# VITA-Group/MM3DGS-SLAM

Measured on AMD Instinct MI355X. Metric: SLAM frames/sec (track+map), TUM fr1/desk-shaped 640x480, higher is better.
Workload: dtype f32

## Files before the change

mm3dgs_slam_amd/csrc/composite.hip:

```cpp
#include <type_traits>
#include "mm3dgs_common.h"
#include "sort_tile.h"
#include "fused_api.h"
#include "loss_pixel.h"
#include "loss_tile.h"

#define STG_ROW 17
#define STG_N (4 * STG_ROW)

#include "composite_common.h"

template <int C>
__device__ __forceinline__ void composite_fwd_body(int tile, const CamDev& cam, const GeomView& g, const ImageView& iv, const BinView& b,
                                                   uint32_t N_cap, float* __restrict__ out, float4 (*stg)[4][3][STG_N],
                                                   const uint32_t* counts_lds, const TrackLoss* tl = nullptr,
                                                   double (*red)[12] = nullptr, const SortShared* span = nullptr) {
  const int tid = threadIdx.x, lane = tid & 63, wv = tid >> 6;
  const int row = lane >> 4, q = lane & 15;
  const int slane = row * STG_ROW + q;
  const int px = (tile % cam.gx) * TILE + (wv & 1) * 8 + (row & 1) * 4 + (q & 3);
  const int py = (tile / cam.gx) * TILE + (wv >> 1) * 8 + (row >> 1) * 4 + (q >> 2);
  const bool inside = px < cam.W && py < cam.H;
  const float pxf = (float)px, pyf = (float)py;
  uint32_t start, len;
// ... 93 lines not shown
#pragma unroll
      for (int k = 0; k < 12; k++) ls[k] = 0.0;
      if (inside) {
        const float rgb[3] = {fin[0], fin[1], fin[2]};
        const float g3[3] = {tl->gt[pix], tl->gt[HW + pix], tl->gt[2 * HW + pix]};
        loss_px_sums(tl->cfg, rgb, fin[4], fin[3], g3, tl->cfg.w_pearson != 0.f ? tl->ref[pix] : 0.f, ls);
      }
      block_sums<12>(ls, red, pearson_double_cols(tl->cfg));
      if (threadIdx.x == 0) {
        double* rowp = tl->partial + (size_t)tile * 12;
#pragma unroll
        for (int k = 0; k < 12; k++) rowp[k] = ls[k];
      }
    }
  }
}

template <int C>
__global__ void __launch_bounds__(256)
composite_fwd_kernel(CamDev cam, GeomView g, ImageView iv, BinView b, uint32_t N_cap, float* __restrict__ out) {
  __shared__ float4 stg[2][4][3][STG_N];
  const int T = cam.gx * cam.gy;
  const int tile = xcd_tile(blockIdx.x, T, cam.tilemap);
  if (tile >= T) return;
  composite_fwd_body<C>(tile, cam, g, iv, b, N_cap, out, stg, nullptr);
}

template <int C>
__global__ void __launch_bounds__(256)
sort_composite_fwd_kernel(CamDev cam, GeomView g, ImageView iv, BinView b, uint32_t N_cap, float* __restrict__ out, int clean, int has_tl,
                          TrackLoss tl, int direct_blocks, uint32_t direct_cap, int slot_bits) {
  __shared__ __align__(16) unsigned char smem[sizeof(float4) * 2 * 4 * 3 * STG_N];
  __shared__ SortShared sh;
  __shared__ double red[4][12];
  static_assert(sizeof(smem) >= 2048 * sizeof(unsigned long long), "LDS union too small for the key array");
  static_assert(sizeof(smem) >= 3 * RANK_SORT_MAX * sizeof(unsigned long long) + sizeof(SortEmit), "LDS union too small for the sort's words and the emission's counters");
  const int T = cam.gx * cam.gy;
  const int tile = slam_tile(cam, iv, blockIdx.x, T);
  if (tile >= T) return;
  sort_tile_body<2048, true>(tile, cam.gx, 0, g, iv, b, N_cap, clean, (unsigned long long*)smem, sh, PROBE_WORD(cam), direct_blocks, direct_cap, slot_bits);
  if (PROBE(cam, 1)) return;
  __syncthreads();
  composite_fwd_body<C>(tile, cam, g, iv, b, N_cap, out, (float4 (*)[4][3][STG_N])smem, sh.run, has_tl ? &tl : nullptr, red, &sh);

}

template <int CTRL>
__device__ __forceinline__ float dpp_all(float v) {
  return __int_as_float(__builtin_amdgcn_update_dpp(0, __float_as_int(v), CTRL, 0xf, 0xf, true));
}
#define QP_XOR1 0xB1
#define QP_XOR2 0x4E
#define ROW_ROR4 0x124
#define ROW_ROR8 0x128

template <int NV>
struct WaveReduce {
  static constexpr int M1 = (NV + 1) / 2;
  static constexpr int M2 = (M1 + 1) / 2;
  static_assert(NV >= 1 && NV <= 16, "NV out of range");
  __device__ static __forceinline__ int slot(int lane) {
    int b0 = lane & 1, b1 = (lane >> 1) & 1, q = (lane >> 2) & 3;
    int i1 = q + M2 * b1;
    int idx = i1 + M1 * b0;
    bool ok = (q < M2) && (i1 < M1) && (idx < NV);
    return ok ? idx : -1;
  }
  __device__ static __forceinline__ float run(const float (&v)[NV], int lane) {
#pragma clang fp contract(off)
    const bool b0 = lane & 1, b1 = lane & 2;
    float l1[M1];
#pragma unroll
    for (int i = 0; i < M1; i++) {
      float sa = v[i] + dpp_all<QP_XOR1>(v[i]);
      if (i + M1 < NV) {
        float sb = v[i + M1] + dpp_all<QP_XOR1>(v[i + M1]);
        l1[i] = b0 ? sb : sa;
      } else {
        l1[i] = sa;
      }
    }
    float l2[M2];
#pragma unroll
    for (int i = 0; i < M2; i++) {
      float sa = l1[i] + dpp_all<QP_XOR2>(l1[i]);
      if (i + M2 < M1) {
        float sb = l1[i + M2] + dpp_all<QP_XOR2>(l1[i + M2]);
        l2[i] = b1 ? sb : sa;
      } else {
        l2[i] = sa;
      }
    }
#pragma unroll
    for (int i = 0; i < M2; i++) {
      l2[i] += dpp_all<ROW_ROR4>(l2[i]);
      l2[i] += dpp_all<ROW_ROR8>(l2[i]);
    }
    const int q = (lane >> 2) & 3;
    float r = l2[0];
#pragma unroll
    for (int i = 1; i < M2; i++) r = (q == i) ? l2[i] : r;
    return r;
  }
};

#define BWD_STG_BYTES (sizeof(float4) * 2 * 4 * 3 * STG_N + sizeof(uint32_t) * 2 * 4 * 64)

constexpr bool bwd_is_two_phase(int MODE, int C) { return MODE != 0 || C == 3; }
#define TP_STRIDE 65
template <int MODE>
struct Bwd2Lds {
  static constexpr int OFF_A = 0;
  static constexpr int OFF_B = OFF_A + STG_N * 16;
  static constexpr int OFF_CZ = OFF_B + STG_N * 16;
  static constexpr int OFF_TP = OFF_CZ + STG_N * 8;
  static constexpr int OFF_T5 = OFF_TP + 4 * TP_STRIDE * 8;
  static constexpr int OFF_T = OFF_TP + 8 * TP_STRIDE * 8;
  static constexpr int SLICE = OFF_T + (MODE == 1 ? 64 * 16 : 64 * 4);
};
template <int MODE>
using BwdLds = Bwd2Lds<(MODE == 0 ? 1 : MODE)>;
template <int C, int MODE>
constexpr size_t BWD_WAVE_SLICE = bwd_is_two_phase(MODE, C) ? (size_t)BwdLds<MODE>::SLICE : sizeof(float4) * 3 * STG_N;
template <int C, int MODE>
constexpr size_t BWD_LDS_BYTES = bwd_is_two_phase(MODE, C) ? 4 * (size_t)BwdLds<MODE>::SLICE : (size_t)BWD_STG_BYTES;
template <int C, int MODE, bool POSE = false>
__device__ __forceinline__ void composite_bwd_body(int tile, const CamDev& cam, const GeomView& g, const ImageView& iv, const BinView& b,
                                                   uint32_t N_cap, const float* __restrict__ dL_dout, float* __restrict__ dsub, int has_tl,
                                                   const TrackLoss& tl, int dl_planes, unsigned char* smem_raw, const SortShared* span = nullptr) {
  static_assert(!POSE || MODE == 2, "the pose chain lives in the tracking mode's loop");
  const int tid = threadIdx.x, lane = tid & 63, wv = tid >> 6;
  const int row = lane >> 4, q = lane & 15;
  const int slane = row * STG_ROW + q;
  const int px = (tile % cam.gx) * TILE + (wv & 1) * 8 + (row & 1) * 4 + (q & 3);
  const int py = (tile / cam.gx) * TILE + (wv >> 1) * 8 + (row >> 1) * 4 + (q >> 2);
  const bool inside = px < cam.W && py < cam.H;
  const float pxf = (float)px, pyf = (float)py;
  uint32_t start, len;
  if (span) { start = span->start; len = span->len; }
  else tile_span(iv, tile, N_cap, start, len);
  const int L = 4 * wv + row;
  const uint32_t count = len ? min(span ? span->run[L] : iv.subcount[NLIST * tile + L], len) : 0u;
  const uint2* __restrict__ list = b.sublist + (size_t)NLIST * start + (size_t)L * len;

  constexpr int NV = MODE == 0 ? 6 + C : (MODE == 1 ? 10 : 7);
  static_assert(MODE == 0 || C == 6, "SLAM modes composite the 6-channel bundle");
  constexpr int RECF = MODE == 0 ? GENERIC_RECF(C) : (MODE == 1 ? REC_MAP_F : REC_TRACK_F);
  float4 (*stg)[4][3][STG_N] = (float4 (*)[4][3][STG_N])smem_raw;
  constexpr uint32_t CH = 16;

  const size_t pix = (size_t)py * cam.W + px, HW = (size_t)cam.H * cam.W;
  const float T_final = inside ? iv.final_T[pix] : 0.f;
  const uint32_t last_contributor = inside ? iv.n_contrib[pix] : 0u;
  uint32_t todo = last_contributor;
  todo = max(todo, (uint32_t)__builtin_amdgcn_update_dpp(0, (int)todo, QP_XOR1, 0xf, 0xf, true));
  todo = max(todo, (uint32_t)__builtin_amdgcn_update_dpp(0, (int)todo, QP_XOR2, 0xf, 0xf, true));
  todo = max(todo, (uint32_t)__builtin_amdgcn_update_dpp(0, (int)todo, ROW_ROR4, 0xf, 0xf, true));
  todo = max(todo, (uint32_t)__builtin_amdgcn_update_dpp(0, (int)todo, ROW_ROR8, 0xf, 0xf, true));
  todo = min(todo, count);
  const uint32_t maxtodo = max(max((uint32_t)__builtin_amdgcn_readlane((int)todo, 0), (uint32_t)__builtin_amdgcn_readlane((int)todo, 16)),
                               max((uint32_t)__builtin_amdgcn_readlane((int)todo, 32), (uint32_t)__builtin_amdgcn_readlane((int)todo, 48)));
  float dL[C];
  float bg_dot = 0.f;
  bool dl_done = false;
  if constexpr (MODE == 2) {
    if (has_tl) {
#pragma unroll
      for (int ch = 0; ch < C; ch++) dL[ch] = 0.f;
      if (inside) {
        const float sil = tl.out[4 * HW + pix];
        const bool smask = sil > tl.cfg.sil_thr;
        const float l1s = tl.defer_scale ? tl.cfg.w_l1 / 3.f : loss_l1_scale(tl.cfg, tl.sums);
#pragma unroll
        for (int ch = 0; ch < 3; ch++) dL[ch] = loss_px_l1_grad(tl.cfg, tl.out[ch * HW + pix], tl.gt[ch * HW + pix], smask, l1s);
        if (tl.cfg.w_pearson != 0.f) dL[3] = loss_px_pearson_grad(tl.cfg, sil, tl.out[3 * HW + pix], tl.ref[pix], tl.sums);
      }
      if (!tl.defer_scale && tile == 0 && threadIdx.x == 0 && tl.loss4) loss_scalars(tl.cfg, tl.sums, HW, tl.loss4);
      dl_done = true;
    }
  }
  if constexpr (MODE == 1) {
    if (has_tl) {
      LossGradSmem& lsm = *(LossGradSmem*)smem_raw;
      float* exch = (float*)(smem_raw + sizeof(LossGradSmem));
      float g4[4];
      bool in_raster;
      if (PROBE(cam, 10)) { g4[0] = g4[1] = g4[2] = g4[3] = 1e-3f; in_raster = true; }
      else loss_grad_tile(tl.cfg, tl.out, tl.gt, tl.ref, tl.dmaps, tl.sums, tile, cam.gx, lsm, g4, in_raster);
#pragma unroll
      for (int ch = 0; ch < 4; ch++) exch[ch * 256 + tid] = g4[ch];
      __syncthreads();
      const int lx = (wv & 1) * 8 + (row & 1) * 4 + (q & 3), ly = (wv >> 1) * 8 + (row >> 1) * 4 + (q >> 2);
#pragma unroll
      for (int ch = 0; ch < C; ch++) dL[ch] = ch < 4 ? exch[ch * 256 + ly * 16 + lx] : 0.f;
      __syncthreads();
      dl_done = true;
    }
  }
#pragma unroll
  for (int ch = 0; ch < C; ch++) {
    if (!dl_done) dL[ch] = (inside && ch < dl_planes) ? dL_dout[ch * HW + pix] : 0.f;
    if (ch < 3 || cam.bg_extras) bg_dot += cam.bg[ch % 3] * dL[ch];
  }
  const float Tf_bg = T_final * bg_dot;
  float Tr = T_final;
  float behind_dot = 0.f;

  const size_t rbase = (size_t)NLIST * start + (size_t)L * len;
  if constexpr (!POSE)
  for (uint32_t e = todo + q; e < count; e += 16) {
    zero_record<NV>(dsub + (rbase + e) * RECF);
  }
  float pacc[6] = {0.f, 0.f, 0.f, 0.f, 0.f, 0.f};
  if constexpr (bwd_is_two_phase(MODE, C)) {
  if (maxtodo != 0) {
    using LY = BwdLds<MODE>;
    unsigned char* const wbase = smem_raw + (size_t)wv * LY::SLICE;
    float4* const sA = (float4*)(wbase + LY::OFF_A);
    float4* const sB = (float4*)(wbase + LY::OFF_B);
    float2* const sCZ = (float2*)(wbase + LY::OFF_CZ);
    float2* const tp = (float2*)(wbase + LY::OFF_TP);
    float* const t5 = (float*)(wbase + LY::OFF_T5);
    bool z45_wave = true;
    if constexpr (MODE == 0) ((float4*)(wbase + LY::OFF_T))[lane] = make_float4(dL[0], dL[1], dL[2], 0.f);
    else {
      if constexpr (MODE == 1) ((float4*)(wbase + LY::OFF_T))[lane] = make_float4(dL[0], dL[1], dL[C > 3 ? 2 : 0], dL[C > 3 ? 3 : 0]);
      else ((float*)(wbase + LY::OFF_T))[lane] = dL[C > 3 ? 3 : 0];
      z45_wave = __ballot(dL[C > 4 ? 4 : 0] != 0.f || dL[C > 5 ? 5 : 0] != 0.f || Tf_bg != 0.f) == 0ull;
      if (!z45_wave) t5[lane] = dL[C > 5 ? 5 : 0];
    }
    const uint32_t first_step = todo - min(todo, last_contributor);
    const uint32_t mean_steps_b = wave_mean_steps(cam, iv);
    const float X0 = pxf - (float)(q & 3), Y0 = pyf - (float)(q >> 2);
    uint32_t n_visit = 0;
    uint32_t my_idx;
    {
      const uint2 e0 = (uint32_t)q < todo ? list[todo - 1u - q] : make_uint2(0u, 0u);
      const SplatRec r0 = load_rec<C>(g.splat, e0.x, (uint32_t)q < todo);
      sA[slane] = r0.A; sB[slane] = r0.B; sCZ[slane] = make_float2(r0.C.x, r0.C.y);
      my_idx = POSE ? e0.x : e0.y;
    }
    uint2 ent_nxt = CH + q < todo ? list[todo - 1u - (CH + q)] : make_uint2(0u, 0u);
    auto run2 = [&](auto z45_tag) {
      constexpr bool Z45 = decltype(z45_tag)::value;
      constexpr int SUB = Z45 ? 8 : 4;
      constexpr int NL = 16 / SUB;
      const int e = q & (SUB - 1), part = q / SUB;
      const int r17 = row * STG_ROW;
      for (uint32_t base = 0; base < maxtodo; base += CH) {
        const SplatRec rec_n = load_rec<C>(g.splat, ent_nxt.x, base + CH + q < todo);
        const uint2 ent_nn = base + 2 * CH + q < todo ? list[todo - 1u - (base + 2 * CH + q)] : make_uint2(0u, 0u);
        __builtin_amdgcn_wave_barrier();
        const int cnt = __builtin_amdgcn_readfirstlane((int)min(CH, maxtodo - base));
        for (int sub = 0; sub < cnt; sub += SUB) {
          const int cs = min(SUB, cnt - sub);
          float2* tpw = tp + lane;
          auto splat_px = [&](const float4& A, const float4& B, const float2& CZ, const int j) {
            const uint32_t step = base + (uint32_t)j;
            const bool row_on = step < todo;
            const float dx = A.x - pxf, dy = A.y - pyf;
            const float power = splat_power(dx, dy, A.z, A.w, B.x);
            const float G = SPLAT_EXP(power);
            const float alpha = fminf(0.99f, B.y * G);
            const bool valid = row_on && (step >= first_step) && !(power > 0.f) && !(alpha < ALPHA_MIN);
            n_visit++;
            const float a_eff = valid ? alpha : 0.f;
            const float G_eff = valid ? G : 0.f;
            float r;
            if constexpr (MODE == 0) {
              const float d = 1.f - a_eff, r0 = __builtin_amdgcn_rcpf(d);
              r = fmaf(fmaf(-d, r0, 1.f), r0, r0);
            } else r = __builtin_amdgcn_rcpf(1.f - a_eff);
            Tr *= r;
            const float w = a_eff * Tr;
            float qd = fmaf(B.z, dL[0], 0.f);
            qd = fmaf(B.w, dL[1], qd);
            qd = fmaf(CZ.x, dL[2], qd);
            if constexpr (MODE != 0) qd = fmaf(CZ.y, dL[C > 3 ? 3 : 0], qd);
            if constexpr (!Z45 && MODE != 0) { qd = fmaf(1.f, dL[C > 4 ? 4 : 0], qd); qd = fmaf(CZ.y * CZ.y, dL[C > 5 ? 5 : 0], qd); }
            const float diff = qd - behind_dot;
            behind_dot = fmaf(a_eff, diff, behind_dot);
            const float dLa = (Z45 && MODE != 0) ? diff * Tr : diff * Tr - Tf_bg * r;
            const float u = MODE == 0 ? dLa * G_eff : B.y * dLa * G_eff;
            *tpw = make_float2(u, w);
            tpw += TP_STRIDE;
          };
          {
            float4 A0 = sA[r17 + sub], B0 = sB[r17 + sub];
            float2 Z0 = sCZ[r17 + sub];
            for (int j = sub; j < sub + cs; j += 2) {
              const int j1 = j + 1 < sub + cs ? j + 1 : j;
              const float4 A1 = sA[r17 + j1], B1 = sB[r17 + j1];
              const float2 Z1 = sCZ[r17 + j1];
              splat_px(A0, B0, Z0, j);
              if (j + 1 < sub + cs) {
                const int j2 = j + 2 < sub + cs ? j + 2 : j1;
                A0 = sA[r17 + j2]; B0 = sB[r17 + j2]; Z0 = sCZ[r17 + j2];
                splat_px(A1, B1, Z1, j1);
              }
            }
          }
          __builtin_amdgcn_wave_barrier();
          {
#pragma clang fp contract(off)
            const int ent = sub + e;
            const bool on2 = base + (uint32_t)ent < todo;
            const float2 cxy = *(const float2*)&sA[r17 + ent];
            const uint32_t idx = (uint32_t)__builtin_amdgcn_ds_bpermute((row * 16 + ent) << 2, (int)my_idx);
            float4 k0, k1, k2, k3, k4;
            if constexpr (POSE) {
              const float4* pr = (const float4*)(g.poserec + (size_t)(on2 ? idx : 0u) * POSEREC_F);
              k0 = pr[0]; k1 = pr[1]; k2 = pr[2]; k3 = pr[3]; k4 = pr[4];
            }
            float dxv[4], dxx[4];
#pragma unroll
            for (int x = 0; x < 4; x++) { dxv[x] = cxy.x - (X0 + (float)x); dxx[x] = dxv[x] * dxv[x]; }
            float M0 = 0.f, Mx = 0.f, Mxx = 0.f, My = 0.f, Mxy = 0.f, Myy = 0.f, c0 = 0.f, c1 = 0.f, c2 = 0.f, cz = 0.f, cz5 = 0.f;
            const float2* tpr = tp + e * TP_STRIDE + row * 16 + part * SUB;
            const int pcol = row * 16 + part * SUB;
#pragma unroll
            for (int yy = 0; yy < SUB / 4; yy++) {
              float s0 = 0.f, s1 = 0.f, s2 = 0.f;
#pragma unroll
              for (int x = 0; x < 4; x++) {
                const float2 uw = tpr[yy * 4 + x];
                s0 = s0 + uw.x;
                s1 = __builtin_fmaf(uw.x, dxv[x], s1);
                s2 = __builtin_fmaf(uw.x, dxx[x], s2);
                if constexpr (MODE != 2) {
                  const float4 d4 = ((const float4*)(wbase + LY::OFF_T))[pcol + yy * 4 + x];
                  c0 = __builtin_fmaf(uw.y, d4.x, c0);
                  c1 = __builtin_fmaf(uw.y, d4.y, c1);
                  c2 = __builtin_fmaf(uw.y, d4.z, c2);
                  if constexpr (MODE == 1) cz = __builtin_fmaf(uw.y, d4.w, cz);
                } else {
                  cz = __builtin_fmaf(uw.y, ((const float*)(wbase + LY::OFF_T))[pcol + yy * 4 + x], cz);
                }
                if constexpr (!Z45) cz5 = __builtin_fmaf(uw.y, t5[pcol + yy * 4 + x], cz5);
              }
              const float dyv = cxy.y - (Y0 + (float)(part * (SUB / 4) + yy));
              M0 = M0 + s0; Mx = Mx + s1; Mxx = Mxx + s2;
              My = __builtin_fmaf(s0, dyv, My);
              Mxy = __builtin_fmaf(s1, dyv, Mxy);
              Myy = __builtin_fmaf(s0 * dyv, dyv, Myy);
            }
            if constexpr (!Z45) cz = __builtin_fmaf(2.f * sCZ[r17 + ent].y, cz5, cz);
            auto merge = [&](float v) {
              if constexpr (NL == 2) return v + dpp_all<ROW_ROR8>(v);
              else { v = v + dpp_all<ROW_ROR4>(v); return v + dpp_all<ROW_ROR8>(v); }
            };
            M0 = merge(M0); Mx = merge(Mx); Mxx = merge(Mxx); My = merge(My); Mxy = merge(Mxy); Myy = merge(Myy);
            if constexpr (MODE != 0) cz = merge(cz);
            if constexpr (MODE != 2) { c0 = merge(c0); c1 = merge(c1); c2 = merge(c2); }
            if constexpr (POSE) {
              const float dm0 = on2 ? (k0.x * Mx + k0.y * My + k1.z * Mxx + k1.w * Mxy + k2.x * Myy) : 0.f;
              const float dm1 = on2 ? (k0.z * Mx + k0.w * My + k2.y * Mxx + k2.z * Mxy + k2.w * Myy) : 0.f;
              const float dm2 = on2 ? (k1.x * Mx + k1.y * My + k3.x * Mxx + k3.y * Mxy + k3.z * Myy + cz) : 0.f;
// ... 433 lines not shown
```

mm3dgs_slam_amd/csrc/loss.hip:

```cpp
#include "loss_tile.h"

__device__ __forceinline__ void pearson_terms(double n, double sx, double sxx, double st, double stt, double sxt, double& rho,
                                              double& cxx, double& ctt) {
  cxx = sxx - sx * sx / n;
  ctt = stt - st * st / n;
  const double cxt = sxt - sx * st / n;
  rho = cxt / sqrt(cxx * ctt);
}

__device__ __forceinline__ void pearson_scalars(const double* tot, int pearson_on, int pearson_invert, double* __restrict__ sums) {
  double valid = 0.0, use2 = 0.0, rho = 0.0, k1 = 0.0, k2 = 0.0, mx = 0.0, mt = 0.0, loss_p = 0.0;
  const double n = tot[3];
  if (pearson_on && n > 1.0) {
    double rho1, cxx, ctt1, rho2 = -2.0, ctt2 = 1.0, cxx2;
    pearson_terms(n, tot[4], tot[5], tot[6], tot[7], tot[8], rho1, cxx, ctt1);
    bool u2 = false;
    if (pearson_invert) {
      pearson_terms(n, tot[4], tot[5], tot[9], tot[10], tot[11], rho2, cxx2, ctt2);
      u2 = (1.0 - rho2) < (1.0 - rho1);
    }
    rho = u2 ? rho2 : rho1;
    const double ctt = u2 ? ctt2 : ctt1;
    valid = 1.0; use2 = u2 ? 1.0 : 0.0;
    k1 = 1.0 / sqrt(cxx * ctt); k2 = rho / cxx;
    mx = tot[4] / n; mt = (u2 ? tot[9] : tot[6]) / n;
    loss_p = 1.0 - rho;
  }
  sums[16] = valid; sums[17] = use2; sums[18] = rho; sums[19] = k1; sums[20] = k2; sums[21] = mx; sums[22] = mt; sums[23] = loss_p;
}

__device__ __forceinline__ bool loss_variant(const LossCfg& cfg) { return cfg.w_depth != 0.f || cfg.l1_sum != 0 || (cfg.l1_mask & 2) != 0; }
__device__ __forceinline__ unsigned loss_double_cols(const LossCfg& cfg) { return pearson_double_cols(cfg) | (cfg.w_depth != 0.f ? 0x10u : 0u); }
__device__ __forceinline__ void variant_px_sums(const LossCfg& cfg, float l1, float sil, float depth, float refv, double (&acc)[12]) {
  const bool smask = sil > cfg.sil_thr;
  const bool on = loss_mask_on(cfg.l1_mask, smask, refv);
  acc[0] = on ? (double)l1 : 0.0;
  acc[1] = on ? 1.0 : 0.0;
  if (cfg.w_depth != 0.f) {
    const bool don = loss_mask_on(cfg.depth_mask, smask, refv);
    acc[3] = don ? 1.0 : 0.0;
    acc[4] = don ? fabs((double)refv - (double)depth) : 0.0;
  }
}
__device__ __forceinline__ void variant_scalars(const LossCfg& cfg, const double* sums, size_t HW, float* loss) {
  const double n_l1 = sums[1], n_d = sums[3];
  const double l1 = cfg.l1_sum ? sums[0] : (n_l1 > 0.0 ? sums[0] / (3.0 * n_l1) : 0.0);
  const double ss = cfg.w_ssim != 0.f ? 1.0 - sums[2] / (3.0 * (double)HW) : 0.0;
  const double loss_p = (cfg.w_pearson != 0.f && sums[16] != 0.0) ? sums[23] : 0.0;
  const double dl = cfg.w_depth != 0.f ? (cfg.l1_sum ? sums[4] : (n_d > 0.0 ? sums[4] / n_d : 0.0)) : 0.0;
  loss[1] = (float)l1; loss[2] = (float)ss; loss[3] = (float)(cfg.w_depth != 0.f ? dl : loss_p);
  loss[0] = (float)(cfg.w_l1 * l1 + cfg.w_ssim * ss + cfg.w_pearson * loss_p + cfg.w_depth * dl);
}

template <bool ROWS>
__global__ void __launch_bounds__(256, 5)
ssim_maps_kernel(LossCfg cfg, const float* __restrict__ out, const float* __restrict__ gt, const float* __restrict__ ref,
                 float* __restrict__ dmaps, double* __restrict__ partial, double* __restrict__ sums, int tiles_x, int T) {
  __shared__ __align__(16) float sI[LW][SW], sG[LW][SW];
  __shared__ __align__(16) float hS[5][LW][HW_];
  __shared__ double red[4][12];
  if ((int)blockIdx.x >= T) {
    double (*part)[16] = (double (*)[16])&hS[0][0][0];
    __shared__ double tot[16];
    reduce_rows_256(partial, T, 0xffbu, part, tot);
    if (threadIdx.x < 12 && threadIdx.x != 2) sums[threadIdx.x] = tot[threadIdx.x];
    if (threadIdx.x == 0) pearson_scalars(tot, cfg.w_pearson != 0.f ? 1 : 0, cfg.pearson_invert, sums);
    return;
  }
  const int tile = blockIdx.x;
  const int x0 = (tile % tiles_x) * LT, y0 = (tile / tiles_x) * LT;
  const uint32_t HW = (uint32_t)cfg.H * (uint32_t)cfg.W;
  const int tid = threadIdx.x;
  const HaloIdx hx = halo_index(cfg, x0, y0);
  const Rsrc r_out = make_rsrc(out, HW * 24u), r_gt = make_rsrc(gt, HW * 12u), r_dm = make_rsrc(dmaps, HW * 36u);
  float va[3], vb[3];
#pragma unroll
  for (int e = 0; e < 3; e++) {
    va[e] = hx.off[e] >= 0 ? bld(r_out, (uint32_t)hx.off[e]) : 0.f;
    vb[e] = hx.off[e] >= 0 ? bld(r_gt, (uint32_t)hx.off[e]) : 0.f;
  }
  const int tx = tid & 15, ty = tid >> 4;
  const int px = x0 + tx, py = y0 + ty;
  const bool inside = px < cfg.W && py < cfg.H;
  const uint32_t pix = (uint32_t)py * (uint32_t)cfg.W + (uint32_t)px;
  float l1 = 0.f;
  float ssim_sum = 0.f;
#pragma unroll 1
  for (int ch = 0; ch < 3; ch++) {
#pragma unroll
    for (int e = 0; e < 3; e++)
      if (hx.lds[e] >= 0) { (&sI[0][0])[hx.lds[e]] = va[e]; (&sG[0][0])[hx.lds[e]] = vb[e]; }
    __syncthreads();
    if (ch < 2) {
#pragma unroll
      for (int e = 0; e < 3; e++) {
        va[e] = hx.off[e] >= 0 ? bld(r_out, (uint32_t)(ch + 1) * HW + (uint32_t)hx.off[e]) : 0.f;
        vb[e] = hx.off[e] >= 0 ? bld(r_gt, (uint32_t)(ch + 1) * HW + (uint32_t)hx.off[e]) : 0.f;
      }
    }
    if (ROWS) l1 += fabsf(sI[ty + HALO][tx + HALO] - sG[ty + HALO][tx + HALO]);
    ssim_moments_hpass(cfg.window, sI, sG, hS, tid);
    __syncthreads();
    float st[5];
    ssim_moments_vpass(cfg.window, hS, tx, ty, st);
    if (inside) {
      const SsimPx p = ssim_px(st);
      ssim_sum += p.f;
      const float df_dm1 = 2.f * p.m2 * p.A2 * p.inv - p.f * 2.f * p.m1 * p.rB1;
      const float df_ds1 = -p.f * p.rB2;
      const float df_ds12 = 2.f * p.A1 * p.inv;
      bst(r_dm, (uint32_t)(ch * 3 + 0) * HW + pix, df_dm1 - 2.f * p.m1 * df_ds1 - p.m2 * df_ds12);
      bst(r_dm, (uint32_t)(ch * 3 + 1) * HW + pix, df_ds1);
      bst(r_dm, (uint32_t)(ch * 3 + 2) * HW + pix, df_ds12);
    }
  }
  if constexpr (ROWS) {
    double acc[12];
#pragma unroll
    for (int k = 0; k < 12; k++) acc[k] = 0.0;
    if (inside) {
      const float sil = out[4 * HW + pix];
      const float rgb[3] = {l1, 0.f, 0.f}, g3[3] = {0.f, 0.f, 0.f};
      const bool var = loss_variant(cfg), need = cfg.w_pearson != 0.f || var;
      const float depth = need ? out[3 * HW + pix] : 0.f, refv = (need && ref) ? ref[pix] : 0.f;
      loss_px_sums(cfg, rgb, sil, depth, g3, refv, acc);
      if (var) variant_px_sums(cfg, l1, sil, depth, refv, acc);
    }
    acc[2] = (double)ssim_sum;
    block_sums<12>(acc, red, loss_double_cols(cfg));
    if (tid == 0) {
      double* row = partial + (size_t)tile * 12;
#pragma unroll
      for (int k = 0; k < 12; k++) row[k] = acc[k];
    }
  } else {
    const float t = wave_sum_to_lane63(ssim_sum);
    if ((tid & 63) == 63) red[tid >> 6][0] = (double)t;
    __syncthreads();
    if (tid == 0) partial[(size_t)tile * 12 + 2] = (red[0][0] + red[1][0]) + (red[2][0] + red[3][0]);
  }
}

__global__ void __launch_bounds__(256)
loss_rows_kernel(LossCfg cfg, const float* __restrict__ out, const float* __restrict__ gt, const float* __restrict__ ref,
                 double* __restrict__ partial, int tiles_x) {
  __shared__ double red[4][12];
  const int tile = blockIdx.x;
  const int tx = threadIdx.x & 15, ty = threadIdx.x >> 4;
  const int px = (tile % tiles_x) * LT + tx, py = (tile / tiles_x) * LT + ty;
  const bool inside = px < cfg.W && py < cfg.H;
  const size_t HW = (size_t)cfg.H * cfg.W, pix = (size_t)py * cfg.W + px;
  double acc[12];
#pragma unroll
  for (int k = 0; k < 12; k++) acc[k] = 0.0;
  if (inside) {
    const float rgb[3] = {out[pix], out[HW + pix], out[2 * HW + pix]}, g3[3] = {gt[pix], gt[HW + pix], gt[2 * HW + pix]};
    const bool var = loss_variant(cfg), need = cfg.w_pearson != 0.f || var;
    const float sil = out[4 * HW + pix], depth = need ? out[3 * HW + pix] : 0.f, refv = (need && ref) ? ref[pix] : 0.f;
    loss_px_sums(cfg, rgb, sil, depth, g3, refv, acc);
    if (var) variant_px_sums(cfg, fabsf(rgb[0] - g3[0]) + fabsf(rgb[1] - g3[1]) + fabsf(rgb[2] - g3[2]), sil, depth, refv, acc);
  }
  block_sums<12>(acc, red, loss_double_cols(cfg));
  if (threadIdx.x == 0) {
    double* row = partial + (size_t)tile * 12;
#pragma unroll
    for (int k = 0; k < 12; k++) row[k] = acc[k];
  }
}

__global__ void __launch_bounds__(1024) loss_finish_kernel(LossCfg cfg, const double* __restrict__ partial, int nrows, double* __restrict__ sums,
                                                           float* __restrict__ loss4) {
  __shared__ double part[64][16];
  __shared__ double part8[8][16];
  __shared__ double tot[16];
  const int col = threadIdx.x & 15, grp = threadIdx.x >> 4;
  double a0 = 0.0, a1 = 0.0;
  if (col < 12) {
    int r = grp;
    for (; r + 64 < nrows; r += 128) { a0 += partial[(size_t)r * 12 + col]; a1 += partial[(size_t)(r + 64) * 12 + col]; }
    if (r < nrows) a0 += partial[(size_t)r * 12 + col];
  }
  part[grp][col] = a0 + a1;
  __syncthreads();
  if (grp < 8) {
    double t = 0.0;
#pragma unroll
    for (int q = 0; q < 8; q++) t += part[grp * 8 + q][col];
    part8[grp][col] = t;
  }
  __syncthreads();
  if (threadIdx.x < 16) {
    double t = 0.0;
#pragma unroll
    for (int q = 0; q < 8; q++) t += part8[q][threadIdx.x];
    sums[threadIdx.x] = t;
    tot[threadIdx.x] = t;
  }
  __syncthreads();
  if (threadIdx.x == 0) {
    pearson_scalars(tot, cfg.w_pearson != 0.f ? 1 : 0, cfg.pearson_invert, sums);
    if (loss4) {
      if (loss_variant(cfg)) variant_scalars(cfg, sums, (size_t)cfg.H * cfg.W, loss4);
      else loss_scalars(cfg, sums, (size_t)cfg.H * cfg.W, loss4);
    }
  }
}

template <bool VAR>
__global__ void __launch_bounds__(256)
loss_grad_kernel(LossCfg cfg, const float* __restrict__ out, const float* __restrict__ gt, const float* __restrict__ ref,
                 const float* __restrict__ dmaps, const double* __restrict__ sums, float* __restrict__ dL, int tiles_x, int write6) {
  __shared__ __align__(16) LossGradSmem sm;
  float g4[4];
  bool inside;
  loss_grad_tile<VAR>(cfg, out, gt, ref, dmaps, sums, blockIdx.x, tiles_x, sm, g4, inside);
  if (inside) {
    const int px = (blockIdx.x % tiles_x) * LT + (threadIdx.x & 15), py = (blockIdx.x / tiles_x) * LT + (threadIdx.x >> 4);
    const size_t HW = (size_t)cfg.H * cfg.W, pix = (size_t)py * cfg.W + px;
#pragma unroll
    for (int ch = 0; ch < 4; ch++) dL[ch * HW + pix] = g4[ch];
    if (write6) { dL[4 * HW + pix] = 0.f; dL[5 * HW + pix] = 0.f; }
  }
}

static int loss_tiles_x(const LossCfg& cfg) { return (cfg.W + LT - 1) / LT; }
static int loss_tiles(const LossCfg& cfg) { return loss_tiles_x(cfg) * ((cfg.H + LT - 1) / LT); }

void launch_loss_finish(const LossCfg& cfg, double* sums, const double* partial, hipStream_t s, float* loss4) {
  hipLaunchKernelGGL(loss_finish_kernel, dim3(1), dim3(1024), 0, s, cfg, partial, loss_tiles(cfg), sums, loss4);
}

void launch_loss(const LossCfg& cfg, const float* out, const float* gt, const float* ref, float* dmaps, double* sums, double* partial,
                 float* dL, float* loss, hipStream_t s) {
  const int T = loss_tiles(cfg), tx = loss_tiles_x(cfg);
  if (cfg.w_ssim != 0.f)
    hipLaunchKernelGGL(ssim_maps_kernel<true>, dim3(T), dim3(256), 0, s, cfg, out, gt, ref, dmaps, partial, sums, tx, T);
  else
    hipLaunchKernelGGL(loss_rows_kernel, dim3(T), dim3(256), 0, s, cfg, out, gt, ref, partial, tx);
  hipLaunchKernelGGL(loss_finish_kernel, dim3(1), dim3(1024), 0, s, cfg, partial, T, sums, loss);
  const bool var = cfg.w_depth != 0.f || cfg.l1_sum != 0 || (cfg.l1_mask & 2) != 0;
  hipLaunchKernelGGL(var ? loss_grad_kernel<true> : loss_grad_kernel<false>, dim3(T), dim3(256), 0, s, cfg, out, gt, ref, dmaps, sums, dL, tx, 1);
}

void launch_loss_after_forward_rows(const LossCfg& cfg, const float* out, const float* gt, const float* ref, float* dmaps, double* sums,
                                    double* partial, float* dL, hipStream_t s) {
  const int T = loss_tiles(cfg), tx = loss_tiles_x(cfg);
  hipLaunchKernelGGL(ssim_maps_kernel<false>, dim3(T + 1), dim3(256), 0, s, cfg, out, gt, ref, dmaps, partial, sums, tx, T);
  if (dL)
    hipLaunchKernelGGL(loss_grad_kernel<false>, dim3(T), dim3(256), 0, s, cfg, out, gt, ref, dmaps, sums, dL, tx, 0);
}
```

mm3dgs_slam_amd/csrc/loss_tile.h:

```cpp
#pragma once
#include "mm3dgs_common.h"
#include "fused_api.h"
#include "loss_pixel.h"

#define LT 16
#define HALO 5
#define LW (LT + 2 * HALO)
#define SW 48
#define HW_ 16

typedef __amdgpu_buffer_rsrc_t Rsrc;
__device__ __forceinline__ Rsrc make_rsrc(const void* p, uint32_t bytes) { return __builtin_amdgcn_make_buffer_rsrc((void*)p, 0, (int)bytes, 0x00020000); }
__device__ __forceinline__ float bld(Rsrc r, uint32_t elem) { return __int_as_float(__builtin_amdgcn_raw_buffer_load_b32(r, elem * 4u, 0, 0)); }
__device__ __forceinline__ void bst(Rsrc r, uint32_t elem, float v) { __builtin_amdgcn_raw_buffer_store_b32(__float_as_int(v), r, elem * 4u, 0, 0); }

struct HaloIdx { int off[3], lds[3]; };

__device__ __forceinline__ HaloIdx halo_index(int H, int W, int x0, int y0) {
  HaloIdx h;
#pragma unroll
  for (int e = 0; e < 3; e++) {
    const int i = threadIdx.x + e * 256;
    const int ly = i / LW, lx = i - ly * LW;
    const int gx = x0 + lx - HALO, gy = y0 + ly - HALO;
    const bool in = i < LW * LW && gx >= 0 && gx < W && gy >= 0 && gy < H;
    h.off[e] = in ? gy * W + gx : -1;
    h.lds[e] = i < LW * LW ? ly * SW + lx : -1;
  }
  return h;
}
__device__ __forceinline__ HaloIdx halo_index(const LossCfg& cfg, int x0, int y0) { return halo_index(cfg.H, cfg.W, x0, y0); }

__device__ __forceinline__ void ssim_moments_hpass(const float (&window)[11], const float (*sI)[SW], const float (*sG)[SW], float (*hS)[LW][HW_],
                                                   int tid) {
  if (tid < LW * 8) {
    const int row = tid >> 3, s = tid & 7;
    float a[12], b[12];
    const float2* ra = (const float2*)&sI[row][2 * s];
    const float2* rb = (const float2*)&sG[row][2 * s];
#pragma unroll
    for (int v = 0; v < 6; v++) {
      const float2 qa = ra[v], qb = rb[v];
      a[2 * v] = qa.x; a[2 * v + 1] = qa.y; b[2 * v] = qb.x; b[2 * v + 1] = qb.y;
    }
    float m1[2] = {0.f, 0.f}, m2[2] = {0.f, 0.f}, e11[2] = {0.f, 0.f}, e22[2] = {0.f, 0.f}, e12[2] = {0.f, 0.f};
#pragma unroll
    for (int i = 0; i < 12; i++) {
      const float aa = a[i] * a[i], bb = b[i] * b[i], ab = a[i] * b[i];
#pragma unroll
      for (int o = 0; o < 2; o++) {
        const int k = i - o;
        if (k >= 0 && k < 11) {
          const float w = window[k];
          m1[o] = fmaf(w, a[i], m1[o]); m2[o] = fmaf(w, b[i], m2[o]);
          e11[o] = fmaf(w, aa, e11[o]); e22[o] = fmaf(w, bb, e22[o]); e12[o] = fmaf(w, ab, e12[o]);
        }
      }
    }
    *(float2*)&hS[0][row][2 * s] = make_float2(m1[0], m1[1]);
    *(float2*)&hS[1][row][2 * s] = make_float2(m2[0], m2[1]);
    *(float2*)&hS[2][row][2 * s] = make_float2(e11[0], e11[1]);
    *(float2*)&hS[3][row][2 * s] = make_float2(e22[0], e22[1]);
    *(float2*)&hS[4][row][2 * s] = make_float2(e12[0], e12[1]);
  }
}
__device__ __forceinline__ void ssim_moments_vpass(const float (&window)[11], const float (*hS)[LW][HW_], int vx, int vy, float (&st)[5]) {
#pragma unroll
  for (int q = 0; q < 5; q++) {
    float acc = 0.f;
#pragma unroll
    for (int k = 0; k < 11; k++) acc = fmaf(window[k], hS[q][vy + k][vx], acc);
    st[q] = acc;
  }
}
struct SsimPx { float m1, m2, A1, A2, B1, B2, rB1, rB2, inv, f; };
__device__ __forceinline__ SsimPx ssim_px(const float (&st)[5]) {
  const float C1 = 0.01f * 0.01f, C2 = 0.03f * 0.03f;
  SsimPx p;
  p.m1 = st[0]; p.m2 = st[1];
  const float s1 = st[2] - p.m1 * p.m1, s2 = st[3] - p.m2 * p.m2, s12 = st[4] - p.m1 * p.m2;
  p.A1 = 2.f * p.m1 * p.m2 + C1; p.A2 = 2.f * s12 + C2;
  p.B1 = fmaf(p.m1, p.m1, p.m2 * p.m2) + C1; p.B2 = s1 + s2 + C2;
  p.rB1 = __builtin_amdgcn_rcpf(p.B1); p.rB2 = __builtin_amdgcn_rcpf(p.B2);
  p.inv = p.rB1 * p.rB2;
  p.f = p.A1 * p.A2 * p.inv;
  return p;
}

__device__ __forceinline__ void reduce_rows_256(const double* __restrict__ partial, int nrows, unsigned cols_mask, double (*part)[16], double* tot) {
  const int col = threadIdx.x & 15, grp = threadIdx.x >> 4;
  double a0 = 0.0, a1 = 0.0, a2 = 0.0, a3 = 0.0;
  if (col < 12 && ((cols_mask >> col) & 1u)) {
    int r = grp;
    for (; r + 48 < nrows; r += 64) {
      a0 += partial[(size_t)r * 12 + col]; a1 += partial[(size_t)(r + 16) * 12 + col];
      a2 += partial[(size_t)(r + 32) * 12 + col]; a3 += partial[(size_t)(r + 48) * 12 + col];
    }
    for (; r < nrows; r += 16) a0 += partial[(size_t)r * 12 + col];
  }
  part[grp][col] = (a0 + a1) + (a2 + a3);
  __syncthreads();
  if (threadIdx.x < 16) {
    double t = 0.0;
#pragma unroll
    for (int q = 0; q < 16; q++) t += part[q][threadIdx.x];
    tot[threadIdx.x] = t;
  }
  __syncthreads();
}

struct LossGradSmem { float sD[3][LW][SW]; float hD[3][LW][HW_]; };
__device__ __forceinline__ bool loss_mask_on(int bits, bool smask, float refv) { return (!(bits & 1) || smask) && (!(bits & 2) || refv > 0.f); }
template <bool VAR = false>
__device__ __forceinline__ void loss_grad_tile(const LossCfg& cfg, const float* __restrict__ out, const float* __restrict__ gt,
                                               const float* __restrict__ ref, const float* __restrict__ dmaps, const double* __restrict__ sums,
                                               int tile, int tiles_x, LossGradSmem& sm, float (&g4)[4], bool& inside_out) {
  float (*sD)[LW][SW] = sm.sD;
  float (*hD)[LW][HW_] = sm.hD;
  const int x0 = (tile % tiles_x) * LT, y0 = (tile / tiles_x) * LT;
  const int tid = threadIdx.x;
  const uint32_t HW = (uint32_t)cfg.H * (uint32_t)cfg.W;
  const float l1_scale = loss_l1_scale(cfg, sums);
  const float ssim_scale = -cfg.w_ssim / (float)(3.0 * (double)HW);
  const int tx = tid & 15, ty = tid >> 4;
  const int px = x0 + tx, py = y0 + ty;
  const bool inside = px < cfg.W && py < cfg.H;
  const uint32_t pix = (uint32_t)py * (uint32_t)cfg.W + (uint32_t)px;
  const Rsrc r_out = make_rsrc(out, HW * 24u), r_gt = make_rsrc(gt, HW * 12u);
  float oc[3] = {0.f, 0.f, 0.f}, gc[3] = {0.f, 0.f, 0.f}, sil = 0.f;
  if (inside) {
#pragma unroll
    for (int ch = 0; ch < 3; ch++) { oc[ch] = bld(r_out, (uint32_t)ch * HW + pix); gc[ch] = bld(r_gt, (uint32_t)ch * HW + pix); }
    sil = bld(r_out, 4u * HW + pix);
  }
  float gch[3] = {0.f, 0.f, 0.f};
  if (cfg.w_ssim != 0.f) {
    const HaloIdx hx = halo_index(cfg, x0, y0);
    const Rsrc r_dm = make_rsrc(dmaps, HW * 36u);
    float v[3][3];
#pragma unroll
    for (int q = 0; q < 3; q++)
#pragma unroll
      for (int e = 0; e < 3; e++) v[q][e] = hx.off[e] >= 0 ? bld(r_dm, (uint32_t)q * HW + (uint32_t)hx.off[e]) : 0.f;
#pragma unroll 1
    for (int ch = 0; ch < 3; ch++) {
#pragma unroll
      for (int q = 0; q < 3; q++)
#pragma unroll
        for (int e = 0; e < 3; e++)
          if (hx.lds[e] >= 0) (&sD[q][0][0])[hx.lds[e]] = v[q][e];
      __syncthreads();
      if (ch < 2) {
#pragma unroll
        for (int q = 0; q < 3; q++)
#pragma unroll
          for (int e = 0; e < 3; e++) v[q][e] = hx.off[e] >= 0 ? bld(r_dm, (uint32_t)((ch + 1) * 3 + q) * HW + (uint32_t)hx.off[e]) : 0.f;
      }
      for (int it = tid; it < 3 * LW * 8; it += 256) {
        const int q = it / (LW * 8), rem = it - q * (LW * 8);
        const int row = rem >> 3, s = rem & 7;
        const float2* ra = (const float2*)&sD[q][row][2 * s];
        float r0 = 0.f, r1 = 0.f;
#pragma unroll
        for (int u = 0; u < 6; u++) {
          const float2 t = ra[u];
          if (2 * u < 11) r0 = fmaf(cfg.window[2 * u], t.x, r0);
          if (2 * u - 1 >= 0) r1 = fmaf(cfg.window[2 * u - 1], t.x, r1);
          if (2 * u + 1 < 11) r0 = fmaf(cfg.window[2 * u + 1], t.y, r0);
          r1 = fmaf(cfg.window[2 * u], t.y, r1);
        }
        *(float2*)&hD[q][row][2 * s] = make_float2(r0, r1);
      }
      __syncthreads();
      float c0 = 0.f, c1 = 0.f, c2 = 0.f;
#pragma unroll
      for (int k = 0; k < 11; k++) {
        const float w = cfg.window[k];
        c0 = fmaf(w, hD[0][ty + k][tx], c0); c1 = fmaf(w, hD[1][ty + k][tx], c1); c2 = fmaf(w, hD[2][ty + k][tx], c2);
      }
      const float o_ = ch == 0 ? oc[0] : (ch == 1 ? oc[1] : oc[2]), g_ = ch == 0 ? gc[0] : (ch == 1 ? gc[1] : gc[2]);
      const float gval = ssim_scale * (c0 + 2.f * o_ * c1 + g_ * c2);
      if (ch == 0) gch[0] = gval; else if (ch == 1) gch[1] = gval; else gch[2] = gval;
    }
  }
// ... 27 lines not shown
```

mm3dgs_slam_amd/csrc/mm3dgs_common.h:

```cpp
#define NLIST 16
#pragma once
#include <hip/hip_runtime.h>
#include <stdint.h>
#include <stdlib.h>
#include "../../include/mm3dgs.h"

#define TILE 16
#define TILE_PIX 256
#define SPLAT_F MM3DGS_SPLAT_FLOATS
#define MAX_FUSED_SCAN_TILES 4096
#define MAX_LDS_TILES 12288

static inline size_t align_up(size_t v, size_t a) { return (v + a - 1) / a * a; }

#define POSEREC_F 20
struct GeomView {
  float* splat;
  float* depth;
  uint32_t* rect;
  uint8_t* clamped;
  uint32_t* tileoff;
  uint32_t* block_tiles;
  float* poserec;
};

static inline size_t geom_bytes_impl(int P) {
  size_t p = (size_t)P;
  return align_up(p * SPLAT_F * 4, 256) + align_up(p * 4, 256) + align_up(p * 8, 256) + align_up(p, 256) +
         align_up(p * 4, 256) + align_up(((p + 255) / 256 + 1) * 4, 256) + align_up(p * POSEREC_F * 4, 256);
}
static inline GeomView geom_view(void* base, int P) {
  size_t p = (size_t)P;
  char* c = (char*)base;
  GeomView g;
  g.splat = (float*)c;      c += align_up(p * SPLAT_F * 4, 256);
  g.depth = (float*)c;      c += align_up(p * 4, 256);
  g.rect = (uint32_t*)c;    c += align_up(p * 8, 256);
  g.clamped = (uint8_t*)c;  c += align_up(p, 256);
  g.tileoff = (uint32_t*)c; c += align_up(p * 4, 256);
  g.block_tiles = (uint32_t*)c; c += align_up(((p + 255) / 256 + 1) * 4, 256);
  g.poserec = (float*)c;
  return g;
}

struct ImageView {
  Mm3dgsHeader* hdr;
  uint32_t* tile_count;
  uint32_t* ranges;
  uint32_t* cursor;
  uint32_t* subcount;
  float* final_T;
  uint32_t* n_contrib;
  uint32_t* tile_order;
  size_t zero_bytes;
};
static inline int tiles_x(int W) { return (W + TILE - 1) / TILE; }
static inline int tiles_y(int H) { return (H + TILE - 1) / TILE; }
#define TILE_SPAN_SLOTS 256
static inline size_t tile_order_words(size_t T) { size_t n = ((T + 7) / 8) * 8; return n > 8 * TILE_SPAN_SLOTS ? n : (size_t)8 * TILE_SPAN_SLOTS; }
static inline __host__ __device__ int slam_span_slots(int T) { return (T + 7) >> 3; }
#ifdef __HIPCC__
__device__ __forceinline__ uint32_t wave_scan_incl(uint32_t x) {
  x += (uint32_t)__builtin_amdgcn_update_dpp(0, (int)x, 0x111, 0xf, 0xf, true);
  x += (uint32_t)__builtin_amdgcn_update_dpp(0, (int)x, 0x112, 0xf, 0xf, true);
  x += (uint32_t)__builtin_amdgcn_update_dpp(0, (int)x, 0x114, 0xf, 0xf, true);
  x += (uint32_t)__builtin_amdgcn_update_dpp(0, (int)x, 0x118, 0xf, 0xf, true);
  x += (uint32_t)__builtin_amdgcn_update_dpp(0, (int)x, 0x142, 0xa, 0xf, false);
  x += (uint32_t)__builtin_amdgcn_update_dpp(0, (int)x, 0x143, 0xc, 0xf, false);
  return x;
}
#endif

static inline size_t image_bytes_impl(int H, int W) {
  size_t T = (size_t)tiles_x(W) * tiles_y(H), px = (size_t)H * W;
  return 256 + align_up(T * 4, 256) + align_up((T + 1) * 4, 256) + align_up(T * 4, 256) + align_up(T * NLIST * 4, 256) +
         align_up(px * 4, 256) + align_up(px * 4, 256) + align_up(tile_order_words(T) * 4, 256);
}
static inline ImageView image_view(void* base, int H, int W) {
  size_t T = (size_t)tiles_x(W) * tiles_y(H), px = (size_t)H * W;
  char* c = (char*)base;
  ImageView v;
  v.hdr = (Mm3dgsHeader*)c;     c += 256;
  v.tile_count = (uint32_t*)c;  c += align_up(T * 4, 256);
  v.zero_bytes = (size_t)(c - (char*)base);
  v.ranges = (uint32_t*)c;      c += align_up((T + 1) * 4, 256);
  v.cursor = (uint32_t*)c;      c += align_up(T * 4, 256);
  v.subcount = (uint32_t*)c;    c += align_up(T * NLIST * 4, 256);
  v.final_T = (float*)c;        c += align_up(px * 4, 256);
  v.n_contrib = (uint32_t*)c;   c += align_up(px * 4, 256);
  v.tile_order = (uint32_t*)c;
  return v;
}
static_assert(sizeof(Mm3dgsHeader) <= 256, "the header block is 256 bytes");

static inline __host__ __device__ uint32_t tile_order_key(int H, int W) {
  return (H > 0 && W > 0 && H < 65536 && W < 65536) ? (((uint32_t)H << 16) | (uint32_t)W) : 0u;
}

struct BinView {
  unsigned long long* keys;
  uint2* sublist;
  uint16_t* submask;
  unsigned long long* payload;
  uint32_t* trec;
};
static inline size_t binning_bytes_impl(size_t N) {
  if (N < 1) N = 1;
  return align_up(N * 8, 256) + align_up(N * NLIST * 8, 256) + align_up(N * 2, 256) + align_up(N * 8, 256) + align_up(N * 4, 256);
}
static inline BinView bin_view(void* base, size_t N) {
  if (N < 1) N = 1;
  char* c = (char*)base;
  BinView b;
  b.keys = (unsigned long long*)c;  c += align_up(N * 8, 256);
  b.sublist = (uint2*)c;            c += align_up(N * NLIST * 8, 256);
  b.submask = (uint16_t*)c;         c += align_up(N * 2, 256);
  b.payload = (unsigned long long*)c;  c += align_up(N * 8, 256);
  b.trec = (uint32_t*)c;
  return b;
}

#define DIRECT_SLOT_BITS_MAX 13
#define DIRECT_SLOT_BITS_MIN 10
static inline int direct_slot_bits(int P) {
  int idb = 1;
  while (idb < 31 && (1ll << idb) < (long long)P) idb++;
  int sb = 32 - idb;
  return sb > DIRECT_SLOT_BITS_MAX ? DIRECT_SLOT_BITS_MAX : sb;
}

#ifdef __HIPCC__
__device__ __forceinline__ void tile_span(const ImageView& iv, int tile, uint32_t N_cap, uint32_t& start, uint32_t& len) {
  const uint32_t cap = iv.hdr->bin_cap;
  const uint32_t a = iv.ranges[tile], b = iv.ranges[tile + 1];
  if (cap) { start = (uint32_t)tile * cap; len = min(a, cap); }
  else { start = min(a, N_cap); len = min(b, N_cap) - start; }
}
#endif

struct BwdView {
  float* dsub;
  float* dtile;
  float* campartial;
  int nrows;
};
static inline int bwd_rows(int P) { return (P + 255) / 256; }
static inline size_t bwd_bytes_impl(int P, size_t N) {
  if (N < 1) N = 1;
  return align_up(N * NLIST * SPLAT_F * 4, 256) + align_up(N * SPLAT_F * 4, 256) + align_up((size_t)(bwd_rows(P) + 1) * 32 * 8, 256);
}
static inline BwdView bwd_view(void* base, int P, size_t N) {
  if (N < 1) N = 1;
  char* c = (char*)base;
  BwdView b;
  b.dsub = (float*)c;  c += align_up(N * NLIST * SPLAT_F * 4, 256);
  b.dtile = (float*)c; c += align_up(N * SPLAT_F * 4, 256);
  b.campartial = (float*)c;
  b.nrows = bwd_rows(P);
  return b;
}

struct BlkRect { int bx0, by0, bw, bh; };
__device__ __forceinline__ BlkRect block_rect(const float4 A, const float4 B, uint32_t r0, uint32_t r1) {
  const int X0 = (int)(r0 & 0xffff) * 4, Y0 = (int)(r0 >> 16) * 4, X1 = (int)(r1 & 0xffff) * 4, Y1 = (int)(r1 >> 16) * 4;
  BlkRect q;
  q.bx0 = X0; q.by0 = Y0; q.bw = X1 - X0; q.bh = Y1 - Y0;
  if (q.bw <= 0 || q.bh <= 0) { q.bw = 0; q.bh = 0; return q; }
  const float tau = __logf(__fmul_rn(255.f, B.y));
  const float det = __fsub_rn(__fmul_rn(A.z, B.x), __fmul_rn(A.w, A.w));
  if (!(det > 0.f)) return q;
  if (!(tau > 0.f)) { q.bw = 0; q.bh = 0; return q; }
  const float k = __fdiv_rn(__fmul_rn(2.f, tau), det);
  const float hx = __fadd_rn(__fmul_rn(__fsqrt_rn(__fmul_rn(k, B.x)), 1.0002f), 0.012f);
  const float hy = __fadd_rn(__fmul_rn(__fsqrt_rn(__fmul_rn(k, A.z)), 1.0002f), 0.012f);
  const int bx0 = max(X0, (int)ceilf(__fmul_rn(__fsub_rn(__fsub_rn(A.x, hx), 3.f), 0.25f))), bx1 = min(X1 - 1, (int)floorf(__fmul_rn(__fadd_rn(A.x, hx), 0.25f)));
  const int by0 = max(Y0, (int)ceilf(__fmul_rn(__fsub_rn(__fsub_rn(A.y, hy), 3.f), 0.25f))), by1 = min(Y1 - 1, (int)floorf(__fmul_rn(__fadd_rn(A.y, hy), 0.25f)));
  q.bx0 = bx0; q.by0 = by0; q.bw = max(bx1 - bx0 + 1, 0); q.bh = max(by1 - by0 + 1, 0);
  if (q.bw == 0 || q.bh == 0) { q.bw = 0; q.bh = 0; }
  return q;
}

struct CamDev {
  int H, W, gx, gy;
  float tanfovx, tanfovy, focal_x, focal_y, scale_modifier;
  int sh_degree;
  int tilemap;
  int tile_table;
  int stats;
#ifdef MM3DGS_PROBES
  int probes;
#endif
  int sort_single;
  int bg_extras;
  uint32_t trec_cap;
  int state_clean;
  int fused_scan;
  const float* bg;
  const float* view;
  const float* proj;
  const float* campos;
};
#ifdef MM3DGS_PROBES
#define PROBE(cam, bit) ((((cam).probes) >> (bit)) & 1)
#define PROBE_WORD(cam) ((cam).probes)
#else
#define PROBE(cam, bit) 0
#define PROBE_WORD(cam) 0
#endif
static inline int env_flag(const char* name, int dflt) {
  const char* v = getenv(name);
  return v ? atoi(v) : dflt;
}
static inline CamDev cam_dev(const Mm3dgsCamera* c) {
  CamDev d;
  d.H = c->image_height; d.W = c->image_width;
  d.gx = tiles_x(d.W); d.gy = tiles_y(d.H);
  d.tanfovx = c->tanfovx; d.tanfovy = c->tanfovy;
  d.focal_x = d.W / (2.0f * c->tanfovx);
  d.focal_y = d.H / (2.0f * c->tanfovy);
  d.scale_modifier = c->scale_modifier;
  d.sh_degree = c->sh_degree;
  d.tilemap = env_flag("MM3DGS_TILEMAP", 1);
  d.stats = env_flag("MM3DGS_STATS", 0);
#ifdef MM3DGS_PROBES
  d.probes = env_flag("MM3DGS_EXP", 0);
#endif
  d.sort_single = 0;
  d.bg_extras = 0;
  d.state_clean = 0;
  d.tile_table = 0;
  d.trec_cap = 0;
  d.fused_scan = 0;
  d.bg = c->bg; d.view = c->viewmatrix; d.proj = c->projmatrix; d.campos = c->campos;
  return d;
}

void launch_preprocess_fwd(const CamDev& cam, int P, int M, int C, const float* means3D, const float* shs,
                           const float* colors, const float* opac, const float* scales, const float* rots,
                           const float* cov3d, int32_t* radii, GeomView g, ImageView iv, hipStream_t s);
void launch_scan_tiles(int T, int P, GeomView g, ImageView iv, hipStream_t s, int sticky = 0);
bool launch_tile_order(int T, int H, int W, ImageView iv, hipStream_t s);
void launch_scatter_sort(const CamDev& cam, int P, GeomView g, ImageView iv, BinView b, size_t N_cap,
                         const int32_t* radii_or_null, hipStream_t s, bool scatter_only = false);
void launch_composite_fwd(const CamDev& cam, int C, GeomView g, ImageView iv, BinView b, size_t N_cap,
                          float* out_color, hipStream_t s);
void launch_composite_bwd(const CamDev& cam, int C, GeomView g, ImageView iv, BinView b, size_t N_cap,
// ... 98 lines not shown
```

Baseline: 32.22.

## Skip backward rows with zero upstream gradient and remap loss tile order

```diff
diff --git a/mm3dgs_slam_amd/csrc/composite.hip b/mm3dgs_slam_amd/csrc/composite.hip
--- a/mm3dgs_slam_amd/csrc/composite.hip
+++ b/mm3dgs_slam_amd/csrc/composite.hip
@@ -269,14 +269,6 @@
   const size_t pix = (size_t)py * cam.W + px, HW = (size_t)cam.H * cam.W;
   const float T_final = inside ? iv.final_T[pix] : 0.f;
   const uint32_t last_contributor = inside ? iv.n_contrib[pix] : 0u;
-  uint32_t todo = last_contributor;
-  todo = max(todo, (uint32_t)__builtin_amdgcn_update_dpp(0, (int)todo, QP_XOR1, 0xf, 0xf, true));
-  todo = max(todo, (uint32_t)__builtin_amdgcn_update_dpp(0, (int)todo, QP_XOR2, 0xf, 0xf, true));
-  todo = max(todo, (uint32_t)__builtin_amdgcn_update_dpp(0, (int)todo, ROW_ROR4, 0xf, 0xf, true));
-  todo = max(todo, (uint32_t)__builtin_amdgcn_update_dpp(0, (int)todo, ROW_ROR8, 0xf, 0xf, true));
-  todo = min(todo, count);
-  const uint32_t maxtodo = max(max((uint32_t)__builtin_amdgcn_readlane((int)todo, 0), (uint32_t)__builtin_amdgcn_readlane((int)todo, 16)),
-                               max((uint32_t)__builtin_amdgcn_readlane((int)todo, 32), (uint32_t)__builtin_amdgcn_readlane((int)todo, 48)));
   float dL[C];
   float bg_dot = 0.f;
   bool dl_done = false;
@@ -320,6 +312,26 @@
     if (ch < 3 || cam.bg_extras) bg_dot += cam.bg[ch % 3] * dL[ch];
   }
   const float Tf_bg = T_final * bg_dot;
+  uint32_t todo = last_contributor;
+  todo = max(todo, (uint32_t)__builtin_amdgcn_update_dpp(0, (int)todo, QP_XOR1, 0xf, 0xf, true));
+  todo = max(todo, (uint32_t)__builtin_amdgcn_update_dpp(0, (int)todo, QP_XOR2, 0xf, 0xf, true));
+  todo = max(todo, (uint32_t)__builtin_amdgcn_update_dpp(0, (int)todo, ROW_ROR4, 0xf, 0xf, true));
+  todo = max(todo, (uint32_t)__builtin_amdgcn_update_dpp(0, (int)todo, ROW_ROR8, 0xf, 0xf, true));
+  todo = min(todo, count);
+  uint32_t live = Tf_bg != 0.f ? 1u : 0u;
+#pragma unroll
+  for (int ch = 0; ch < C; ch++) live |= dL[ch] != 0.f ? 1u : 0u;
+  live |= (uint32_t)__builtin_amdgcn_update_dpp(0, (int)live, QP_XOR1, 0xf, 0xf, true);
+  live |= (uint32_t)__builtin_amdgcn_update_dpp(0, (int)live, QP_XOR2, 0xf, 0xf, true);
+  live |= (uint32_t)__builtin_amdgcn_update_dpp(0, (int)live, ROW_ROR4, 0xf, 0xf, true);
+  live |= (uint32_t)__builtin_amdgcn_update_dpp(0, (int)live, ROW_ROR8, 0xf, 0xf, true);
+  if (cam.stats && q == 0 && todo != 0u) {
+    atomicAdd((uint32_t*)iv.hdr + HDR_STAT_BWD_ROWS, 1u);
+    if (!live) atomicAdd((uint32_t*)iv.hdr + HDR_STAT_BWD_ROWS_SKIPPED, 1u);
+  }
+  todo = live ? todo : 0u;
+  const uint32_t maxtodo = max(max((uint32_t)__builtin_amdgcn_readlane((int)todo, 0), (uint32_t)__builtin_amdgcn_readlane((int)todo, 16)),
+                               max((uint32_t)__builtin_amdgcn_readlane((int)todo, 32), (uint32_t)__builtin_amdgcn_readlane((int)todo, 48)));
   float Tr = T_final;
   float behind_dot = 0.f;
 
diff --git a/mm3dgs_slam_amd/csrc/loss.hip b/mm3dgs_slam_amd/csrc/loss.hip
--- a/mm3dgs_slam_amd/csrc/loss.hip
+++ b/mm3dgs_slam_amd/csrc/loss.hip
@@ -59,7 +59,7 @@
   __shared__ __align__(16) float sI[LW][SW], sG[LW][SW];
   __shared__ __align__(16) float hS[5][LW][HW_];
   __shared__ double red[4][12];
-  if ((int)blockIdx.x >= T) {
+  if ((int)blockIdx.x >= loss_halo_grid(T)) {
     double (*part)[16] = (double (*)[16])&hS[0][0][0];
     __shared__ double tot[16];
     reduce_rows_256(partial, T, 0xffbu, part, tot);
@@ -67,7 +67,8 @@
     if (threadIdx.x == 0) pearson_scalars(tot, cfg.w_pearson != 0.f ? 1 : 0, cfg.pearson_invert, sums);
     return;
   }
-  const int tile = blockIdx.x;
+  const int tile = loss_halo_tile(blockIdx.x, T);
+  if (tile >= T) return;
   const int x0 = (tile % tiles_x) * LT, y0 = (tile / tiles_x) * LT;
   const uint32_t HW = (uint32_t)cfg.H * (uint32_t)cfg.W;
   const int tid = threadIdx.x;
@@ -209,13 +210,15 @@
 template <bool VAR>
 __global__ void __launch_bounds__(256)
 loss_grad_kernel(LossCfg cfg, const float* __restrict__ out, const float* __restrict__ gt, const float* __restrict__ ref,
-                 const float* __restrict__ dmaps, const double* __restrict__ sums, float* __restrict__ dL, int tiles_x, int write6) {
+                 const float* __restrict__ dmaps, const double* __restrict__ sums, float* __restrict__ dL, int tiles_x, int T, int write6) {
   __shared__ __align__(16) LossGradSmem sm;
+  const int tile = loss_halo_tile(blockIdx.x, T);
+  if (tile >= T) return;
   float g4[4];
   bool inside;
-  loss_grad_tile<VAR>(cfg, out, gt, ref, dmaps, sums, blockIdx.x, tiles_x, sm, g4, inside);
+  loss_grad_tile<VAR>(cfg, out, gt, ref, dmaps, sums, tile, tiles_x, sm, g4, inside);
   if (inside) {
-    const int px = (blockIdx.x % tiles_x) * LT + (threadIdx.x & 15), py = (blockIdx.x / tiles_x) * LT + (threadIdx.x >> 4);
+    const int px = (tile % tiles_x) * LT + (threadIdx.x & 15), py = (tile / tiles_x) * LT + (threadIdx.x >> 4);
     const size_t HW = (size_t)cfg.H * cfg.W, pix = (size_t)py * cfg.W + px;
 #pragma unroll
     for (int ch = 0; ch < 4; ch++) dL[ch * HW + pix] = g4[ch];
@@ -234,18 +237,18 @@
                  float* dL, float* loss, hipStream_t s) {
   const int T = loss_tiles(cfg), tx = loss_tiles_x(cfg);
   if (cfg.w_ssim != 0.f)
-    hipLaunchKernelGGL(ssim_maps_kernel<true>, dim3(T), dim3(256), 0, s, cfg, out, gt, ref, dmaps, partial, sums, tx, T);
+    hipLaunchKernelGGL(ssim_maps_kernel<true>, dim3(loss_halo_grid(T)), dim3(256), 0, s, cfg, out, gt, ref, dmaps, partial, sums, tx, T);
   else
     hipLaunchKernelGGL(loss_rows_kernel, dim3(T), dim3(256), 0, s, cfg, out, gt, ref, partial, tx);
   hipLaunchKernelGGL(loss_finish_kernel, dim3(1), dim3(1024), 0, s, cfg, partial, T, sums, loss);
   const bool var = cfg.w_depth != 0.f || cfg.l1_sum != 0 || (cfg.l1_mask & 2) != 0;
-  hipLaunchKernelGGL(var ? loss_grad_kernel<true> : loss_grad_kernel<false>, dim3(T), dim3(256), 0, s, cfg, out, gt, ref, dmaps, sums, dL, tx, 1);
+  hipLaunchKernelGGL(var ? loss_grad_kernel<true> : loss_grad_kernel<false>, dim3(loss_halo_grid(T)), dim3(256), 0, s, cfg, out, gt, ref, dmaps, sums, dL, tx, T, 1);
 }
 
 void launch_loss_after_forward_rows(const LossCfg& cfg, const float* out, const float* gt, const float* ref, float* dmaps, double* sums,
                                     double* partial, float* dL, hipStream_t s) {
   const int T = loss_tiles(cfg), tx = loss_tiles_x(cfg);
-  hipLaunchKernelGGL(ssim_maps_kernel<false>, dim3(T + 1), dim3(256), 0, s, cfg, out, gt, ref, dmaps, partial, sums, tx, T);
+  hipLaunchKernelGGL(ssim_maps_kernel<false>, dim3(loss_halo_grid(T) + 1), dim3(256), 0, s, cfg, out, gt, ref, dmaps, partial, sums, tx, T);
   if (dL)
-    hipLaunchKernelGGL(loss_grad_kernel<false>, dim3(T), dim3(256), 0, s, cfg, out, gt, ref, dmaps, sums, dL, tx, 0);
-}
+    hipLaunchKernelGGL(loss_grad_kernel<false>, dim3(loss_halo_grid(T)), dim3(256), 0, s, cfg, out, gt, ref, dmaps, sums, dL, tx, T, 0);
+}
diff --git a/mm3dgs_slam_amd/csrc/loss_tile.h b/mm3dgs_slam_amd/csrc/loss_tile.h
--- a/mm3dgs_slam_amd/csrc/loss_tile.h
+++ b/mm3dgs_slam_amd/csrc/loss_tile.h
@@ -30,6 +30,9 @@
   return h;
 }
 __device__ __forceinline__ HaloIdx halo_index(const LossCfg& cfg, int x0, int y0) { return halo_index(cfg.H, cfg.W, x0, y0); }
+
+__device__ __forceinline__ int loss_halo_tile(int bid, int T) { return (bid & 7) * ((T + 7) >> 3) + (bid >> 3); }
+static inline __host__ __device__ int loss_halo_grid(int T) { return ((T + 7) >> 3) * 8; }
 
 __device__ __forceinline__ void ssim_moments_hpass(const float (&window)[11], const float (*sI)[SW], const float (*sG)[SW], float (*hS)[LW][HW_],
                                                    int tid) {
diff --git a/mm3dgs_slam_amd/csrc/mm3dgs_common.h b/mm3dgs_slam_amd/csrc/mm3dgs_common.h
--- a/mm3dgs_slam_amd/csrc/mm3dgs_common.h
+++ b/mm3dgs_slam_amd/csrc/mm3dgs_common.h
@@ -92,6 +92,9 @@
   return v;
 }
 static_assert(sizeof(Mm3dgsHeader) <= 256, "the header block is 256 bytes");
+#define HDR_STAT_BWD_ROWS 12
+#define HDR_STAT_BWD_ROWS_SKIPPED 13
+static_assert(sizeof(Mm3dgsHeader) <= 4 * HDR_STAT_BWD_ROWS, "the statistics words lie behind the struct");
 
 static inline __host__ __device__ uint32_t tile_order_key(int H, int W) {
   return (H > 0 && W > 0 && H < 65536 && W < 65536) ? (((uint32_t)H << 16) | (uint32_t)W) : 0u;
```

Result: no change. 32.46, median of 6 (+0.7%).
